# google-research/frame-interpolation

Hardware: NVIDIA H100
Metric: interpolated_frames_per_sec_1080p (higher is better)
Workload: dtype f16x2-split (activations/weights as fp16 hi+lo planes; fp32 accumulate)

## Files before the change

### frame_interpolation_b200/csrc/film_conv.h

```cpp
#pragma once
#include <cuda.h>
#include <stdint.h>

#include "film_common.cuh"

namespace film {

constexpr int kMaxSrc = 4;
constexpr int kMaxTaps = 9;
constexpr int kChunk = 64;
constexpr int kTileM = 128;

struct ConvSrc {
  const sp_t* hi;
  const sp_t* lo;
  int C;
  int c_off;
  int nchunk;
  int bswap;
};

struct alignas(64) ConvProblem {
  CUtensorMap tm_a_hi[kMaxSrc];
  CUtensorMap tm_a_lo[kMaxSrc];
  CUtensorMap tm_w_hi;
  CUtensorMap tm_w_lo;
  CUtensorMap tm_w_hi_half;
  CUtensorMap tm_w_lo_half;
  ConvSrc src[kMaxSrc];
  int nsrc;
  int B, H, W;
  int tile_h, tile_w;
  int tiles_y, tiles_x;
  int ntaps;
  int tap_dy[kMaxTaps], tap_dx[kMaxTaps];
  int kchunk;
  int ktot;
  const sp_t* w_hi;
  const sp_t* w_lo;
  const float* bias;
  int cout;
  int act;
  sp_t* out_hi;
  sp_t* out_lo;
  int out_C, out_c_off;
  int out_H, out_W;
  int out_sy, out_sx, out_oy, out_ox;
  int epi_mode;
  const float* head_w3;
  const float* head_b3;
  int crop_y, crop_x, crop_h, crop_w;
  int64_t crop_pitch;
  const float* head_w4;
  const float* head_b4;
  const float* head_vup;
  float* head_res;
  float* head_v;
  int v2_resident;
  int v2_na, v2_nw;
  int v2_grid;
  int v2_part_lo, v2_part_hi;
  sp_t* pool_hi;
  sp_t* pool_lo;
  int pool_C;
  int group;
  int pair;
  int halo;
  int bn;
  int passes;
  int straight;
  int out_lo_skip;
  int pxn;
};

cudaError_t launch_conv_tc(const ConvProblem* d_prob, const ConvProblem& h_prob, cudaStream_t st);
cudaError_t launch_conv_simt(const ConvProblem* d_prob, const ConvProblem& h_prob, cudaStream_t st);
cudaError_t conv_tc_configure();
bool conv3x3_tc_plan(ConvProblem& h_prob, int num_sms);
void conv3x3_tc_pick_tile(int H, int W, int B, int cout, int kc, int passes, int ktot, int epi_mode, int num_sms,
                          int& tile_h, int& tile_w);
cudaError_t launch_conv3x3_tc(const ConvProblem* d_prob, const ConvProblem& h_prob, cudaStream_t st);
cudaError_t conv3x3_tc_configure();
}
```

### frame_interpolation_b200/csrc/film_conv3x3_tc.cu

```cuda
#include <cuda.h>
#include <cuda_runtime.h>
#include <stdint.h>

#include <type_traits>

#include "film_conv.h"
#include "film_tc_ptx.cuh"

namespace film {
namespace {
using namespace tc;

constexpr int kConsumers = 256;
constexpr int kThreads = kConsumers + 128;
__host__ __device__ constexpr int a_plane_bytes(int kc, int th, int tw) { return (th + 2) * tw * kc * 2; }
__host__ __device__ constexpr int a_stage_bytes(int kc, int th, int tw) { return 2 * a_plane_bytes(kc, th, tw); }
constexpr int kHaloW = 10;
__host__ __device__ constexpr int halo_box_bytes(int kc, int th) { return (th + 2) * kHaloW * kc * 2; }
__host__ __device__ constexpr int halo_plane_bytes(int kc, int th) { return (halo_box_bytes(kc, th) + 1023) & ~1023; }
__host__ __device__ constexpr int a_stage_bytes_h(int kc, int th, int tw, int halo, int planes = 2) {
  return planes * (halo ? halo_plane_bytes(kc, th) : a_plane_bytes(kc, th, tw));
}
constexpr int kMaxRing = 8;
constexpr int kSmemLimit = 227 * 1024;
constexpr int kBarBytes = 8 * (4 * kMaxRing + 4);
constexpr int kFixedBytes = kBarBytes + 16 + 512 * 4  + 64  + 1024  + 64;
constexpr int kHeadW3 = 64 * 32 * 4, kHeadMisc = 512;
constexpr int kHeadBytes = kHeadW3 + kHeadMisc;
constexpr int kPxnStageWg = 64 * 64 * 2;
constexpr int kPxnStageBytes = 2 * kPxnStageWg;
constexpr int kFoldLd = 136;
constexpr int kFoldStageWg = 32 * kFoldLd * 4;
inline int epi_scratch_bytes(int epi_mode, int pxn, int bn) {
  if (pxn && bn == 32) return (epi_mode == 3 ? kHeadBytes : 0) + 2 * kFoldStageWg;
  return epi_mode == 3 ? kHeadBytes : pxn ? kPxnStageBytes : 0;
}

__host__ __device__ constexpr int w_rows(int bn, int pxn) { return pxn && bn == 32 ? 64 : bn; }
__host__ __device__ inline int w_tap_bytes(int bn, int kc, int planes = 2) { return bn * kc * 2 * planes; }

template <int BN, int KC, bool kPartial, bool kHalo, bool kOne, bool kRes, bool kPxN = false>
__global__ void __launch_bounds__(kThreads, 1) k_conv3x3_tc(const ConvProblem* __restrict__ prob) {
  static_assert(!kPxN || ((BN == 64 || BN == 128) && KC == 64) || (BN == 32 && kOne && !kPartial),
                "pixels on N: one or two M = 64 weight tiles of 64-channel chunks, or the folded single-pass Cout = 32 form");
  extern __shared__ uint8_t smem_raw[];
  constexpr bool one = kOne;
  const int planes = one ? 1 : 2;
  constexpr bool kFold = kPxN && BN == 32;
  constexpr int kWPlane = w_rows(BN, kPxN) * KC * 2;
  const int kWTap = kWPlane * planes;
  const int kTileH = prob->tile_h, kTileW = prob->tile_w;
  constexpr int kHaloTileH = kPxN ? 32 : 16;
  constexpr int kHaloBox = halo_box_bytes(KC, kHaloTileH), kHaloPlane = halo_plane_bytes(KC, kHaloTileH);
  constexpr bool halo = kHalo;
  const int kAPlane = halo ? kHaloPlane : a_plane_bytes(KC, kTileH, kTileW);
  const int kAStage = planes * kAPlane;
  const int kRowStep = kTileW * KC * 2;
  constexpr bool kFused = BN <= 128 && !kPxN;
  constexpr int kMh = kPxN && !kFold ? BN / 64 : 1;
  constexpr int kPxnN = kFold ? 136 : 128;
  constexpr int kAccRegs = kPxN ? kPxnN / 2 * kMh : (kFused ? 2 * BN : BN) / 2;
  constexpr int kWgPx = kPxN ? 128 : 64;

  const int NA = prob->v2_na, NW = prob->v2_nw;
  const bool resident = prob->v2_resident != 0;
  const int nsrc = prob->nsrc;
  const int tiles_x = prob->tiles_x, tiles_per_img = prob->tiles_y * prob->tiles_x;
  const int cout = prob->cout;
  const int n_nt = (cout + BN - 1) / BN;
  const int ntiles = prob->B * tiles_per_img * n_nt;
  constexpr int kStageTaps = kHalo ? 9 : 3;
  constexpr int kStageMmas = kFold ? 2 * kStageTaps / 3 : kStageTaps;
  constexpr bool kPacked = kPartial && kPxN;
  const int part_lo = prob->v2_part_lo, part_hi = prob->v2_part_hi;
  int nab = 0;
  for (int s = 0; s < nsrc; ++s) nab += prob->src[s].nchunk * (kHalo ? 1 : 3);
  const int nkb = nab * kStageMmas - (kPacked ? (part_hi - part_lo) * (kStageTaps - kStageTaps / 3) : 0);

  const FastDiv div_nt(n_nt, ntiles), div_img(tiles_per_img, ntiles), div_tx(tiles_x, ntiles);
  const bool pair = prob->pair != 0;
  const int rank = pair ? (int)cluster_ctarank() : 0;
  const int nsp = prob->B * tiles_per_img;
  const int nwork = pair ? ((nsp + 1) / 2) * n_nt : ntiles;
  const int w_first = pair ? (int)blockIdx.x >> 1 : (int)blockIdx.x, w_step = pair ? (int)gridDim.x >> 1 : (int)gridDim.x;
  auto decode = [&](int work, int& sp, int& nti) {
    div_nt.divmod(work, sp, nti);
    if (pair) sp = 2 * sp + rank;
  };

  const uint32_t raw = smem_u32(smem_raw);
  const uint32_t base = (raw + 1023u) & ~1023u;
  uint8_t* gen_base = smem_raw + (base - raw);
  const uint32_t a_base = base;
  const uint32_t w_base = a_base + (uint32_t)NA * kAStage;
  const uint32_t w_bytes = resident ? (uint32_t)nkb * kWTap : (uint32_t)NW * kWTap;
  const uint32_t tail = w_base + w_bytes;
  const uint32_t tail_off = (uint32_t)NA * kAStage + w_bytes;
  float* bias_smem = reinterpret_cast<float*>(gen_base + tail_off + kBarBytes + 16);
  int* src_tab = reinterpret_cast<int*>(gen_base + tail_off + kBarBytes + 16 + 512 * 4);

  const int warp = threadIdx.x >> 5, lane = threadIdx.x & 31;

  if (warp == 8 && lane == 0) {
    for (int s = 0; s < kMaxRing; ++s) {
      mbar_init(tail + 8u * s, 1);
      mbar_init(tail + 8u * (kMaxRing + s), 2);
      mbar_init(tail + 8u * (2 * kMaxRing + s), 1);
      mbar_init(tail + 8u * (3 * kMaxRing + s), pair ? 4 : 2);
    }
    for (int s = 0; s < kMaxSrc; ++s) {
      src_tab[2 * s] = s < nsrc ? prob->src[s].nchunk : 0;
      src_tab[2 * s + 1] = s < nsrc ? prob->src[s].c_off : 0;
      src_tab[2 * kMaxSrc + s] = s < nsrc ? prob->src[s].bswap : 0;
    }
    asm volatile("fence.mbarrier_init.release.cluster;" ::: "memory");
  }
  if (warp < 8)
    for (int i = threadIdx.x; i < n_nt * BN; i += kConsumers) bias_smem[i] = (i < cout) ? prob->bias[i] : 0.f;
  __syncthreads();
  if (pair) cluster_sync_all();
  auto leave = [&]() {
    if (pair) cluster_sync_all();
  };

  if (warp >= 8) {
    regs_dec<40>();
    if (warp > 8) {
      leave();
      return;
    }
    const CUtensorMap* tm_w_hi = &prob->tm_w_hi;
    const CUtensorMap* tm_w_lo = &prob->tm_w_lo;
    if (resident && elect_one()) {
      mbar_expect_tx(tail + 8u * (2 * kMaxRing), (uint32_t)nkb * kWTap);
      for (int kb = 0; kb < nkb; ++kb) {
        tma_load_2d(w_base + kb * kWTap, tm_w_hi, tail + 8u * (2 * kMaxRing), kb * KC, 0);
        if (!one) tma_load_2d(w_base + kb * kWTap + kWPlane, tm_w_lo, tail + 8u * (2 * kMaxRing), kb * KC, 0);
      }
    }
    __syncwarp();
    RingPos ra, rw;
    for (int tile = w_first; tile < nwork; tile += w_step) {
      int sp, nti, b, rem, ty, tx;
      decode(tile, sp, nti);
      div_img.divmod(sp, b, rem);
      div_tx.divmod(rem, ty, tx);
      const int n0 = nti * BN, y0 = ty * kTileH, x0 = tx * kTileW;
      {
        const int nt = tile + w_step;
        int next_sp, nnt;
        decode(nt < nwork ? nt : 0, next_sp, nnt);
        if (nt < nwork && next_sp != sp && next_sp < nsp && elect_one()) {
          int nb, nrem, nty, ntx;
          div_img.divmod(next_sp, nb, nrem);
          div_tx.divmod(nrem, nty, ntx);
          const int ny0 = nty * kTileH, nx0 = ntx * kTileW;
          for (int s = 0; s < nsrc; ++s)
            for (int ch = 0; ch < src_tab[2 * s]; ++ch) {
              const int cc = src_tab[2 * s + 1] + ch * KC;
              tma_prefetch_4d(&prob->tm_a_hi[s], cc, nx0 - 1, ny0 - 1, nb);
              if (!one) tma_prefetch_4d(&prob->tm_a_lo[s], cc, nx0 - 1, ny0 - 1, nb);
              if (!halo) {
                tma_prefetch_4d(&prob->tm_a_hi[s], cc, nx0 + 1, ny0 - 1, nb);
                if (!one) tma_prefetch_4d(&prob->tm_a_lo[s], cc, nx0 + 1, ny0 - 1, nb);
              }
            }
        }
        __syncwarp();
      }
      int kb = 0, ab = 0;
      for (int s = 0; s < nsrc; ++s) {
        const int nchunk = src_tab[2 * s], c_off = src_tab[2 * s + 1];
        const int bs = src_tab[2 * kMaxSrc + s] ? prob->B - 1 - b : b;
        const CUtensorMap* tm_hi = &prob->tm_a_hi[s];
        const CUtensorMap* tm_lo = &prob->tm_a_lo[s];
        for (int ch = 0; ch < nchunk; ++ch) {
          const int nst = halo ? 1 : 3;
          for (int dx = 0; dx < nst; ++dx, ++ab) {
            const int st = ra.stage;
            mbar_wait(tail + 8u * (kMaxRing + st), ra.phase ^ 1u);
            if (elect_one()) {
              const uint32_t sa = a_base + st * kAStage, bar = tail + 8u * st;
              mbar_expect_tx(bar, halo ? (uint32_t)(planes * kHaloBox) : (uint32_t)kAStage);
              tma_load_4d(sa, tm_hi, bar, c_off + ch * KC, x0 + dx - 1, y0 - 1, bs);
              if (!one) tma_load_4d(sa + kAPlane, tm_lo, bar, c_off + ch * KC, x0 + dx - 1, y0 - 1, bs);
            }
            __syncwarp();
            ra.advance(NA);
            if (!resident) {
              const bool packed = kPacked && ab >= part_lo && ab < part_hi;
              const int nblk = packed ? kStageTaps / 3 : kStageMmas;
              for (int t = 0; t < nblk; ++t, ++kb) {
                const int ws = rw.stage;
                mbar_wait(tail + 8u * (3 * kMaxRing + ws), rw.phase ^ 1u);
                if (elect_one()) {
                  const uint32_t sw = w_base + ws * kWTap, bar = tail + 8u * (2 * kMaxRing + ws);
                  mbar_expect_tx(bar, kWTap);
                  if (pair) {
                    const uint32_t hoff = (uint32_t)(rank * (kWPlane / 2));
                    tma_load_2d_mc(sw + hoff, &prob->tm_w_hi_half, bar, kb * KC, n0 + rank * (BN / 2), 3);
                    if (!one) tma_load_2d_mc(sw + kWPlane + hoff, &prob->tm_w_lo_half, bar, kb * KC, n0 + rank * (BN / 2), 3);
                  } else {
                    tma_load_2d(sw, tm_w_hi, bar, kb * KC, n0);
                    if (!one) tma_load_2d(sw + kWPlane, tm_w_lo, bar, kb * KC, n0);
                  }
                }
                __syncwarp();
                rw.advance(NW);
              }
            }
          }
        }
      }
    }
    leave();
    return;
  }

  regs_inc<232>();
  const int wg = warp >> 2;
  const int q = lane & 3;
  const int H = prob->H, W = prob->W, out_H = prob->out_H, out_W = prob->out_W, out_C = prob->out_C;
  const int out_c_off = prob->out_c_off, act = prob->act;
  sp_t* const out_hi = prob->out_hi;
  sp_t* const out_lo = prob->out_lo;
  sp_t* const pool_hi = prob->pool_hi;
  sp_t* const pool_lo = prob->pool_lo;
  const int pool_C = prob->pool_C;
  const bool do_pool = pool_hi != nullptr;
  const bool lo_skip = prob->out_lo_skip != 0;
  const bool rgb = prob->epi_mode == 2;
  const float* const head_w = prob->head_w4;
  float* const rgb_out = prob->head_v;
  const int crop_y = prob->crop_y, crop_x = prob->crop_x, crop_h = prob->crop_h, crop_w = prob->crop_w;
  const int64_t crop_pitch = prob->crop_pitch;
  const bool fhead = prob->epi_mode == 3;
  constexpr int kHid = BN <= 64 ? BN / 2 : 1;
  float* const w3s = reinterpret_cast<float*>(reinterpret_cast<uint8_t*>(src_tab) + 64);
  float* const hmisc = w3s + kHeadW3 / 4;
  if (fhead) {
    if constexpr (BN <= 64) {
      for (int i = threadIdx.x; i < BN * kHid; i += kConsumers) w3s[i] = prob->head_w3[i];
      for (int i = threadIdx.x; i < kHid; i += kConsumers) hmisc[i] = prob->head_b3[i];
      for (int i = threadIdx.x; i < 2 * kHid; i += kConsumers) hmisc[kHid + i] = prob->head_w4[i];
      if (threadIdx.x < 2) hmisc[3 * kHid + threadIdx.x] = prob->head_b4[threadIdx.x];
    }
    asm volatile("bar.sync 1, %0;" ::"r"(kConsumers) : "memory");
  }
  const float* const head_vup = prob->head_vup;
  float* const head_res = prob->head_res;
  float* const head_vout = prob->head_v;

  if (resident) mbar_wait(tail + 8u * (2 * kMaxRing), 0);
  const bool is_leader = (threadIdx.x & 127) == 0;
  const uint32_t w_empty_peer = pair ? map_to_cta(tail + 8u * (3 * kMaxRing), (uint32_t)(rank ^ 1)) : 0u;
  auto release_w = [&](int slot) {
    mbar_arrive(tail + 8u * (3 * kMaxRing + slot));
    if (pair) mbar_arrive_cluster(w_empty_peer + 8u * slot);
  };
  {
    constexpr int kWTapC = kWPlane * (kOne ? 1 : 2);
    constexpr uint32_t kPx = KC * 2;
    const uint32_t a_row0 = kHalo ? (uint32_t)(wg * (kWgPx / 8) * kHaloW) * kPx : (uint32_t)(wg * kWgPx) * kPx;
    const uint32_t sbo = kHalo ? kHaloW * kPx : 8 * kPx;
    RingPos ra, rw;
    float acc[kAccRegs];
    auto tap_of = [](int m) { return kFold ? (kHalo ? 3 * (m / 2) : 0) + m % 2 : m; };
    auto pxn_mma = [&](uint64_t w_hi, uint64_t w_lo, uint64_t a_hi, uint64_t a_lo, uint32_t accf) {
#pragma unroll
      for (int h = 0; h < kMh; ++h) {
        const uint64_t wh = (uint64_t)(h * (64 * KC * 2) >> 4);
        wgmma<kPxnN>(acc + 64 * h, w_hi + wh, a_hi, accf);
        if constexpr (!kOne) {
          wgmma<kPxnN>(acc + 64 * h, w_lo + wh, a_hi, 1u);
          wgmma<kPxnN>(acc + 64 * h, w_hi + wh, a_lo, 1u);
        }
      }
    };
    for (int tile = w_first; tile < nwork; tile += w_step) {
      int kb = 0;
      int rel_a = -1, rel_w = -1;
      auto retire = [&](int next_a, int next_w) {
        wgmma_commit();
        wgmma_wait<1>();
        if (is_leader) {
          if (rel_a >= 0) mbar_arrive(tail + 8u * (kMaxRing + rel_a));
          if (rel_w >= 0) release_w(rel_w);
        }
        rel_a = next_a;
        rel_w = next_w;
      };
      auto stage = [&](auto ksteps_c, auto tpb_c) {
        constexpr int kSteps = decltype(ksteps_c)::value, kTpb = decltype(tpb_c)::value;
        constexpr int kBlocks = kStageMmas / kTpb;
        const int st = ra.stage;
        mbar_wait(tail + 8u * st, ra.phase);
        const uint32_t sa = a_base + st * kAStage + a_row0;
        const uint32_t lo_off = (uint32_t)(kHalo ? kHaloPlane : kAPlane);
        if constexpr (kRes) {
          const uint64_t a0 = make_desc_sbo<KC>(sa, sbo);
          const uint64_t lo_delta = (uint64_t)(lo_off >> 4);
          const uint64_t row_delta = (uint64_t)(kRowStep >> 4);
          const uint64_t w0 = make_desc_kc<KC>(w_base + kb * kWTapC);
          const uint32_t first = (kb == 0) ? 0u : 1u;
          wgmma_fence();
#pragma unroll
          for (int mi = 0; mi < kStageMmas; ++mi) {
            const int t = tap_of(mi);
            const uint64_t a_hi = a0 + (kHalo ? (uint64_t)((((t % 3) * kHaloW + t / 3) * kPx) >> 4) : (uint64_t)t * row_delta);
            const uint64_t a_lo = a_hi + lo_delta;
            const uint64_t w_hi = w0 + (uint64_t)(((mi / kTpb) * kWTapC + (mi % kTpb) * kSteps * 32) >> 4);
            const uint64_t w_lo = w_hi + (uint64_t)(kWPlane >> 4);
#pragma unroll
            for (int k = 0; k < kSteps; ++k) {
              const uint64_t adv = (uint64_t)(k * 32 >> 4);
              const uint32_t accf = (mi == 0 && k == 0) ? first : 1u;
              if constexpr (kPxN) {
                pxn_mma(w_hi + adv, w_lo + adv, a_hi + adv, a_lo + adv, accf);
              } else if constexpr (kOne) {
                wgmma<BN>(acc, a_hi + adv, w_hi + adv, accf);
              } else if constexpr (kFused) {
                wgmma<BN>(acc, a_hi + adv, w_hi + adv, accf);
                wgmma<BN>(acc + BN / 2, a_hi + adv, w_lo + adv, accf);
                wgmma<BN>(acc, a_lo + adv, w_hi + adv, 1u);
              } else {
                wgmma<BN>(acc, a_lo + adv, w_hi + adv, accf);
                wgmma<BN>(acc, a_hi + adv, w_lo + adv, 1u);
                wgmma<BN>(acc, a_hi + adv, w_hi + adv, 1u);
              }
            }
          }
          retire(st, -1);
          kb += kBlocks;
        } else {
          for (int blk = 0; blk < kBlocks; ++blk, ++kb) {
            uint32_t sw;
            int ws = -1;
            if (resident) {
              sw = w_base + kb * kWTap;
            } else {
              ws = rw.stage;
              mbar_wait(tail + 8u * (2 * kMaxRing + ws), rw.phase);
              sw = w_base + ws * kWTap;
            }
            const uint32_t first = (kb == 0) ? 0u : 1u;
            wgmma_fence();
#pragma unroll
            for (int u = 0; u < kTpb; ++u) {
              const int t = tap_of(blk * kTpb + u);
              const uint32_t off = kHalo ? (uint32_t)((t % 3) * kHaloW + t / 3) * kPx : (uint32_t)(t * kRowStep);
              const uint64_t a_hi = make_desc_sbo<KC>(sa + off, sbo);
              const uint64_t a_lo = make_desc_sbo<KC>(sa + lo_off + off, sbo);
              const uint64_t wk = (uint64_t)((u * kSteps * 32) >> 4);
              const uint64_t w_hi = make_desc_kc<KC>(sw) + wk, w_lo = make_desc_kc<KC>(sw + kWPlane) + wk;
#pragma unroll
              for (int k = 0; k < kSteps; ++k) {
                const uint64_t adv = (uint64_t)(k * 32 >> 4);
                const uint32_t accf = (u == 0 && k == 0) ? first : 1u;
                if constexpr (kPxN) {
                  pxn_mma(w_hi + adv, w_lo + adv, a_hi + adv, a_lo + adv, accf);
                } else if constexpr (kOne) {
                  wgmma<BN>(acc, a_hi + adv, w_hi + adv, accf);
                } else if constexpr (kFused) {
                  wgmma<BN>(acc, a_hi + adv, w_hi + adv, accf);
                  wgmma<BN>(acc + BN / 2, a_hi + adv, w_lo + adv, accf);
                  wgmma<BN>(acc, a_lo + adv, w_hi + adv, 1u);
                } else {
                  wgmma<BN>(acc, a_lo + adv, w_hi + adv, accf);
                  wgmma<BN>(acc, a_hi + adv, w_lo + adv, 1u);
                  wgmma<BN>(acc, a_hi + adv, w_hi + adv, 1u);
                }
              }
            }
            retire(blk == kBlocks - 1 ? st : -1, ws);
            if (!resident) rw.advance(NW);
          }
        }
        ra.advance(NA);
      };
      using Full = std::integral_constant<int, KC / 16>;
      using One = std::integral_constant<int, 1>;
      if constexpr (kPartial) {
        for (int ab = 0; ab < part_lo; ++ab) stage(Full{}, One{});
        for (int ab = part_lo; ab < part_hi; ++ab) stage(One{}, std::integral_constant<int, kPacked ? 3 : 1>{});
        for (int ab = part_hi; ab < nab; ++ab) stage(Full{}, One{});
      } else {
        for (int ab = 0; ab < nab; ++ab) stage(Full{}, One{});
      }
      wgmma_wait<0>();
      if (is_leader) {
        if (rel_a >= 0) mbar_arrive(tail + 8u * (kMaxRing + rel_a));
        if (rel_w >= 0) release_w(rel_w);
      }
      acc_fence<kAccRegs>(acc);

      int sp, nti, b, rem, ty, tx;
      decode(tile, sp, nti);
      div_img.divmod(sp, b, rem);
      div_tx.divmod(rem, ty, tx);
      const int n0 = nti * BN;
      const bool live = sp < nsp;
      if constexpr (kFold) {
        float* const stg = reinterpret_cast<float*>(reinterpret_cast<uint8_t*>(src_tab) + 64 + (fhead ? kHeadBytes : 0) +
                                                    wg * kFoldStageWg);
        auto wg_sync = [&]() { asm volatile("bar.sync %0, 128;" ::"r"(2 + wg) : "memory"); };
        const bool lower = (warp & 2) != 0;
        const int r0 = 16 * (warp & 1) + (lane >> 2);
        wg_sync();
        if (!lower) {
#pragma unroll
          for (int j = 0; j < 16; ++j)
#pragma unroll
            for (int h = 0; h < 2; ++h)
              *reinterpret_cast<float2*>(stg + (r0 + 8 * h) * kFoldLd + 8 * j + 2 * q) =
                  make_float2(acc[4 * j + 2 * h], acc[4 * j + 2 * h + 1]);
        }
        wg_sync();
        if (lower) {
#pragma unroll
          for (int j = 1; j < 17; ++j)
#pragma unroll
            for (int h = 0; h < 2; ++h) {
              float2* d = reinterpret_cast<float2*>(stg + (r0 + 8 * h) * kFoldLd + 8 * (j - 1) + 2 * q);
              const float2 v = *d;
              *d = make_float2(v.x + acc[4 * j + 2 * h], v.y + acc[4 * j + 2 * h + 1]);
            }
        }
        wg_sync();
        const int p = threadIdx.x & 127;
        const int py = ty * kTileH + 16 * wg + (p >> 3), px = tx * kTileW + (p & 7);
        const int64_t opix = ((int64_t)b * out_H + py) * out_W + px;
        float f[32];
#pragma unroll
        for (int c = 0; c < 32; ++c) {
          const float x = stg[c * kFoldLd + p] + bias_smem[c];
          f[c] = act ? leaky(x) : x;
        }
        if (!live || py >= H || px >= W) {
        } else if (fhead) {
          float hp[16];
#pragma unroll
          for (int hh = 0; hh < 16; ++hh) hp[hh] = 0.f;
#pragma unroll
          for (int c = 0; c < 32; ++c) {
            const float4* wr = reinterpret_cast<const float4*>(w3s + c * 16);
#pragma unroll
            for (int h4 = 0; h4 < 4; ++h4) {
              const float4 wv = wr[h4];
              hp[4 * h4] = fmaf(f[c], wv.x, hp[4 * h4]);
              hp[4 * h4 + 1] = fmaf(f[c], wv.y, hp[4 * h4 + 1]);
              hp[4 * h4 + 2] = fmaf(f[c], wv.z, hp[4 * h4 + 2]);
              hp[4 * h4 + 3] = fmaf(f[c], wv.w, hp[4 * h4 + 3]);
            }
          }
          float f0 = hmisc[3 * 16], f1 = hmisc[3 * 16 + 1];
#pragma unroll
          for (int hh = 0; hh < 16; ++hh) {
            const float x = leaky(hp[hh] + hmisc[hh]);
            f0 = fmaf(x, hmisc[16 + 2 * hh], f0);
            f1 = fmaf(x, hmisc[16 + 2 * hh + 1], f1);
          }
          float2 res = make_float2(f0, f1), tot = res;
          if (head_vup) {
            const float2 u = reinterpret_cast<const float2*>(head_vup)[opix];
            tot.x += u.x;
            tot.y += u.y;
          }
          reinterpret_cast<float2*>(head_res)[opix] = res;
// ... 153 lines not shown
            for (int e = 0; e < 2; ++e) {
              const int c = n0 + 8 * j + 2 * q + e;
              float f = value(h, j, e) + bias_smem[c];
              if (act) f = leaky(f);
              r0 = fmaf(f, __ldg(head_w + 3 * c), r0);
              r1 = fmaf(f, __ldg(head_w + 3 * c + 1), r1);
              r2 = fmaf(f, __ldg(head_w + 3 * c + 2), r2);
            }
#pragma unroll
          for (int m = 1; m <= 2; m <<= 1) {
            r0 += __shfl_xor_sync(0xffffffffu, r0, m);
            r1 += __shfl_xor_sync(0xffffffffu, r1, m);
            r2 += __shfl_xor_sync(0xffffffffu, r2, m);
          }
          const int oy = py - crop_y, ox = px - crop_x;
          if (q == 0 && valid && oy >= 0 && oy < crop_h && ox >= 0 && ox < crop_w) {
            float* o = rgb_out + (int64_t)oy * crop_pitch + (int64_t)ox * 3;
            o[0] = r0 + __ldg(prob->head_b4);
            o[1] = r1 + __ldg(prob->head_b4 + 1);
            o[2] = r2 + __ldg(prob->head_b4 + 2);
          }
        }
      }
      if (!fhead && !rgb) {
        bool valid[2];
        int64_t opix[2];
#pragma unroll
        for (int h = 0; h < 2; ++h) {
          const int r = wg * 64 + (warp & 3) * 16 + (lane >> 2) + 8 * h;
          const int py = ty * kTileH + r / kTileW, px = tx * kTileW + r % kTileW;
          valid[h] = live && (py < H) && (px < W);
          opix[h] = ((int64_t)b * out_H + py) * out_W + px;
        }
        const int r0 = wg * 64 + (warp & 3) * 16 + (lane >> 2);
        const int py0 = ty * kTileH + r0 / kTileW, px0 = tx * kTileW + r0 % kTileW;
        const bool pool_ok = live && (py0 >> 1) < (out_H >> 1) && (px0 >> 1) < (out_W >> 1) && !(lane & 4);
        const int64_t ppix = ((int64_t)b * (out_H >> 1) + (py0 >> 1)) * (out_W >> 1) + (px0 >> 1);
#pragma unroll
        for (int j = 0; j < BN / 8; ++j) {
          const int c = 8 * j + 2 * q;
          if (n0 + c >= cout) break;
          float a[2][2];
#pragma unroll
          for (int h = 0; h < 2; ++h) {
            float f0 = value(h, j, 0) + bias_smem[n0 + c], f1 = value(h, j, 1) + bias_smem[n0 + c + 1];
            if (act) {
              f0 = leaky(f0);
              f1 = leaky(f1);
            }
            if (valid[h]) {
              sp_t* oh = out_hi + opix[h] * out_C + out_c_off + n0;
              if (lo_skip) {
                *reinterpret_cast<uint32_t*>(oh + c) = pack2_hi(f0, f1);
              } else {
                sp_t* ol = out_lo + opix[h] * out_C + out_c_off + n0;
                uint32_t hi, lo;
                split_pack2(f0, f1, hi, lo);
                *reinterpret_cast<uint32_t*>(oh + c) = hi;
                *reinterpret_cast<uint32_t*>(ol + c) = lo;
              }
            }
            if (do_pool) {
              a[h][0] = f0 + __shfl_xor_sync(0xffffffffu, f0, 4);
              a[h][1] = f1 + __shfl_xor_sync(0xffffffffu, f1, 4);
            }
          }
          if (do_pool && pool_ok) {
            uint32_t hi, lo;
            split_pack2((a[0][0] + a[1][0]) * 0.25f, (a[0][1] + a[1][1]) * 0.25f, hi, lo);
            *reinterpret_cast<uint32_t*>(pool_hi + ppix * pool_C + n0 + c) = hi;
            *reinterpret_cast<uint32_t*>(pool_lo + ppix * pool_C + n0 + c) = lo;
          }
        }
      }
    }
  }
  leave();
}

int smem_bytes_for(const ConvProblem& h, int bn) {
  const int nkb = h.ktot / h.kchunk;
  const int planes = h.passes == 1 ? 1 : 2;
  const int wtap = w_tap_bytes(w_rows(bn, h.pxn), h.kchunk, planes);
  const int w = h.v2_resident ? nkb * wtap : h.v2_nw * wtap;
  return h.v2_na * a_stage_bytes_h(h.kchunk, h.tile_h, h.tile_w, h.halo, planes) + w + kFixedBytes +
         epi_scratch_bytes(h.epi_mode, h.pxn, bn);
}

}

int conv_tc_block_n(int cout);

namespace {
bool ring_depths(int kc, int tile_h, int tile_w, int halo, int planes, int bn, int cout, int ktot, int epi_mode, int pxn,
                 int& resident, int& na, int& nw) {
  const int wtap = w_tap_bytes(w_rows(bn, pxn), kc, planes);
  const int w_all = (ktot / kc) * wtap;
  const int kLimit = kSmemLimit - epi_scratch_bytes(epi_mode, pxn, bn);
  const int kAStage = a_stage_bytes_h(kc, tile_h, tile_w, halo, planes);
  if (cout <= bn && w_all + 2 * kAStage + kFixedBytes <= kLimit) {
    resident = 1;
    const int n = (kLimit - kFixedBytes - w_all) / kAStage;
    const int n_max = halo ? 3 : 6;
    na = n > n_max ? n_max : n;
    nw = 1;
    return true;
  }
  resident = 0;
  na = halo ? 2 : (bn >= 128 ? 2 : 3);
  int n = (kLimit - kFixedBytes - na * kAStage) / wtap;
  if (n < 2 && na > 2) {
    na = 2;
    n = (kLimit - kFixedBytes - na * kAStage) / wtap;
  }
  nw = n > kMaxRing ? kMaxRing : n;
  return nw >= 2;
}
}

void conv3x3_tc_pick_tile(int H, int W, int B, int cout, int kc, int passes, int ktot, int epi_mode, int num_sms,
                          int& tile_h, int& tile_w) {
  static const int cand[3][2] = {{16, 8}, {8, 16}, {4, 32}};
  const int bn = conv_tc_block_n(cout);
  const int n_nt = (cout + bn - 1) / bn;
  double best = 1e30;
  tile_h = 16;
  tile_w = 8;
  for (auto& c : cand) {
    int res, na, nw;
    if (!ring_depths(kc, c[0], c[1], 0, passes == 1 ? 1 : 2, bn, cout, ktot, epi_mode, 0, res, na, nw)) continue;
    const long tiles = (long)B * ((H + c[0] - 1) / c[0]) * ((W + c[1] - 1) / c[1]) * n_nt;
    const long waves = (tiles + num_sms - 1) / num_sms;
    const double cost = (double)waves * (c[0] + 2.0) / c[0] * (1.0 + 1e-3 * (c[1] / 8));
    if (cost < best) {
      best = cost;
      tile_h = c[0];
      tile_w = c[1];
    }
  }
}

bool conv3x3_tc_plan(ConvProblem& h, int num_sms) {
  const int bn = h.bn;
  const int planes = h.passes == 1 ? 1 : 2;
  const int wtap = w_tap_bytes(w_rows(bn, h.pxn), h.kchunk, planes);
  const int w_all = (h.ktot / h.kchunk) * wtap;
  const bool can_resident = h.cout <= bn;
  const int kLimit = kSmemLimit - epi_scratch_bytes(h.epi_mode, h.pxn, bn);
  if (h.halo && (h.tile_h != (h.pxn ? 32 : 16) || h.tile_w != 8 ||
                 (can_resident && w_all + 2 * a_stage_bytes_h(h.kchunk, h.tile_h, h.tile_w, 0, planes) + kFixedBytes <= kLimit &&
                  w_all + 2 * a_stage_bytes_h(h.kchunk, h.tile_h, h.tile_w, 1, planes) + kFixedBytes > kLimit)))
    h.halo = 0;
  bool ok = ring_depths(h.kchunk, h.tile_h, h.tile_w, h.halo, planes, bn, h.cout, h.ktot, h.epi_mode, h.pxn,
                        h.v2_resident, h.v2_na, h.v2_nw);
  if (!ok && h.halo) {
    h.halo = 0;
    ok = ring_depths(h.kchunk, h.tile_h, h.tile_w, 0, planes, bn, h.cout, h.ktot, h.epi_mode, h.pxn, h.v2_resident,
                     h.v2_na, h.v2_nw);
  }
  const int nsp = h.B * h.tiles_y * h.tiles_x, n_nt = (h.cout + bn - 1) / bn;
  if (h.pair) {
    const int nwork = (nsp + 1) / 2 * n_nt, nclu = num_sms / 2;
    h.v2_grid = 2 * (nwork < nclu ? nwork : nclu);
  } else {
    h.v2_grid = nsp * n_nt < num_sms ? nsp * n_nt : num_sms;
  }
  return ok;
}

using ConvKernel = void (*)(const ConvProblem*);
template <int BN, int KC, bool kPartial, bool kHalo, bool kOne, bool kRes, bool kPxN>
constexpr ConvKernel kernel_of() {
  if constexpr (kPxN && BN == 32 && (kPartial || !kOne))
    return nullptr;
  else
    return k_conv3x3_tc<BN, KC, kPartial, kHalo, kOne, kRes, kPxN>;
}

template <int BN, int KC, bool kPxN = false>
struct Variants {
  static constexpr ConvKernel kFn[16] = {
      kernel_of<BN, KC, false, false, false, false, kPxN>(), kernel_of<BN, KC, false, false, false, true, kPxN>(),
      kernel_of<BN, KC, false, false, true, false, kPxN>(),  kernel_of<BN, KC, false, false, true, true, kPxN>(),
      kernel_of<BN, KC, false, true, false, false, kPxN>(),  kernel_of<BN, KC, false, true, false, true, kPxN>(),
      kernel_of<BN, KC, false, true, true, false, kPxN>(),   kernel_of<BN, KC, false, true, true, true, kPxN>(),
      kernel_of<BN, KC, true, false, false, false, kPxN>(),  kernel_of<BN, KC, true, false, false, true, kPxN>(),
      kernel_of<BN, KC, true, false, true, false, kPxN>(),   kernel_of<BN, KC, true, false, true, true, kPxN>(),
      kernel_of<BN, KC, true, true, false, false, kPxN>(),   kernel_of<BN, KC, true, true, false, true, kPxN>(),
      kernel_of<BN, KC, true, true, true, false, kPxN>(),    kernel_of<BN, KC, true, true, true, true, kPxN>()};
  static cudaError_t configure() {
    for (auto fn : kFn) {
      if (!fn) continue;
      const cudaError_t e = cudaFuncSetAttribute(fn, cudaFuncAttributeMaxDynamicSharedMemorySize, kSmemLimit);
      if (e != cudaSuccess) return e;
    }
    return cudaSuccess;
  }
  static cudaError_t launch(const ConvProblem* d_prob, const ConvProblem& h, cudaStream_t st) {
    if (h.v2_na < 2 || (!h.v2_resident && h.v2_nw < 2)) return cudaErrorInvalidValue;
    if (kPxN && (h.pair || h.tile_h != 32 || h.tile_w != 8 || h.epi_mode != (BN == 32 && h.epi_mode == 3 ? 3 : 0)))
      return cudaErrorInvalidValue;
    if (kPxN && BN == 32 && h.pool_hi) return cudaErrorInvalidValue;
    const bool partial = h.v2_part_hi > h.v2_part_lo;
    const int idx = (partial ? 8 : 0) | (h.halo ? 4 : 0) | (h.passes == 1 ? 2 : 0) | (h.v2_resident && h.straight ? 1 : 0);
    if (!kFn[idx]) return cudaErrorInvalidValue;
    if (!h.pair) {
      kFn[idx]<<<h.v2_grid, kThreads, smem_bytes_for(h, BN), st>>>(d_prob);
      return cudaGetLastError();
    }
    cudaLaunchConfig_t cfg = {};
    cudaLaunchAttribute attr[1];
    attr[0].id = cudaLaunchAttributeClusterDimension;
    attr[0].val.clusterDim.x = 2;
    attr[0].val.clusterDim.y = 1;
    attr[0].val.clusterDim.z = 1;
    cfg.gridDim = dim3(h.v2_grid);
    cfg.blockDim = dim3(kThreads);
    cfg.dynamicSmemBytes = smem_bytes_for(h, BN);
    cfg.stream = st;
    cfg.attrs = attr;
    cfg.numAttrs = 1;
    return cudaLaunchKernelEx(&cfg, kFn[idx], d_prob);
  }
};

cudaError_t conv3x3_tc_configure() {
  cudaError_t e;
#define FILM_CFG(BN, KC)                        \
  e = Variants<BN, KC>::configure();            \
  if (e != cudaSuccess) return e;
  FILM_CFG(32, 64) FILM_CFG(64, 64) FILM_CFG(128, 64) FILM_CFG(256, 64) FILM_CFG(32, 32) FILM_CFG(64, 32)
#undef FILM_CFG
  e = Variants<64, 64, true>::configure();
  if (e != cudaSuccess) return e;
  e = Variants<128, 64, true>::configure();
  if (e != cudaSuccess) return e;
  e = Variants<32, 64, true>::configure();
  if (e != cudaSuccess) return e;
  e = Variants<32, 32, true>::configure();
  if (e != cudaSuccess) return e;
  return cudaSuccess;
}

cudaError_t launch_conv3x3_tc(const ConvProblem* d_prob, const ConvProblem& h, cudaStream_t st) {
  const int bn = h.bn;
  if (h.kchunk == 32) {
    if (bn == 32) return h.pxn ? Variants<32, 32, true>::launch(d_prob, h, st) : Variants<32, 32>::launch(d_prob, h, st);
    if (bn == 64) return Variants<64, 32>::launch(d_prob, h, st);
    return cudaErrorInvalidValue;
  }
  switch (bn) {
    case 256: return Variants<256, 64>::launch(d_prob, h, st);
    case 128: return h.pxn ? Variants<128, 64, true>::launch(d_prob, h, st) : Variants<128, 64>::launch(d_prob, h, st);
    case 64: return h.pxn ? Variants<64, 64, true>::launch(d_prob, h, st) : Variants<64, 64>::launch(d_prob, h, st);
    default: return h.pxn ? Variants<32, 64, true>::launch(d_prob, h, st) : Variants<32, 64>::launch(d_prob, h, st);
  }
}

}
```

### frame_interpolation_b200/csrc/film_kernels.cu

```cuda
#include "film_conv.h"
#include "film_kernels.h"

namespace film {

static inline int cdiv(int64_t a, int64_t b) { return (int)((a + b - 1) / b); }

__device__ __forceinline__ uint4 ldg16(const void* p) { return __ldg(reinterpret_cast<const uint4*>(p)); }

__global__ void k_image_pool(const float* __restrict__ in, float* __restrict__ out, int B, int H,
                             int W) {
  const int Ho = H / 2, Wo = W / 2;
  const int64_t n = (int64_t)B * Ho * Wo * 3;
  int64_t i = (int64_t)blockIdx.x * blockDim.x + threadIdx.x;
  if (i >= n) return;
  int c = (int)(i % 3);
  int64_t p = i / 3;
  int x = (int)(p % Wo);
  p /= Wo;
  int y = (int)(p % Ho);
  int b = (int)(p / Ho);
  const float* r0 = in + (((int64_t)b * H + 2 * y) * W + 2 * x) * 3 + c;
  const float* r1 = r0 + (int64_t)W * 3;
  out[i] = (r0[0] + r0[3] + r1[0] + r1[3]) * 0.25f;
}
// ... 185 lines not shown
  float acc[8];
#pragma unroll
  for (int j = 0; j < 8; ++j) acc[j] = 0.f;
#pragma unroll
  for (int ky = 0; ky < 3; ++ky) {
    int yy = y + ky - 1;
    if (yy < 0 || yy >= H) continue;
#pragma unroll
    for (int kx = 0; kx < 3; ++kx) {
      int xx = x + kx - 1;
      if (xx < 0 || xx >= W) continue;
      const float* ip = img + (((int64_t)b * H + yy) * W + xx) * 3;
#pragma unroll
      for (int ci = 0; ci < 3; ++ci) {
        float v = __ldg(ip + ci);
        const float* wr = ws + ((ky * 3 + kx) * 3 + ci) * 64 + g * 8;
#pragma unroll
        for (int j = 0; j < 8; ++j) acc[j] = fmaf(v, wr[j], acc[j]);
      }
    }
  }
#pragma unroll
  for (int j = 0; j < 8; ++j) acc[j] = leaky(acc[j] + bs[g * 8 + j]);
  uint4 h, l;
  pack8(acc, h, l);
  int64_t o = p * out_C + out_c_off + g * 8;
  *reinterpret_cast<uint4*>(out_hi + o) = h;
  *reinterpret_cast<uint4*>(out_lo + o) = l;
}

constexpr int kC0H = 8, kC0W = 16;
constexpr int kC0Tiles = 4;
constexpr int kC0Patch = (kC0H + 2) * (kC0W + 2) * 3;
constexpr int kC0PatchRegs = (kC0Patch + 127) / 128;
__device__ __forceinline__ float fe_patch_load(const float* __restrict__ img, int b, int H, int W, int y0, int x0, int i) {
  const int c = i % 3, px = (i / 3) % (kC0W + 2), py = i / (3 * (kC0W + 2));
  const int yy = y0 + py - 1, xx = x0 + px - 1;
  return (i < kC0Patch && yy >= 0 && yy < H && xx >= 0 && xx < W) ? __ldg(img + (((int64_t)b * H + yy) * W + xx) * 3 + c) : 0.f;
}
__global__ void __launch_bounds__(128) k_fe_conv0(const float* __restrict__ img, int H, int W,
                                                  const float* __restrict__ w, const float* __restrict__ bias,
                                                  sp_t* __restrict__ out_hi, sp_t* __restrict__ out_lo, int lo_skip,
                                                  float* __restrict__ pool_out) {
  __shared__ float4 ws[27 * 16];
  __shared__ float bs[64];
  __shared__ float patch[kC0Patch];
  const int tid = threadIdx.x;
  const int b = blockIdx.z, y0 = blockIdx.y * kC0H, xb = blockIdx.x * (kC0W * kC0Tiles);
  for (int i = tid; i < 27 * 16; i += 128) ws[i] = __ldg(reinterpret_cast<const float4*>(w) + i);
  if (tid < 64) bs[tid] = bias[tid];
  float nxt[kC0PatchRegs];
#pragma unroll
  for (int j = 0; j < kC0PatchRegs; ++j) nxt[j] = fe_patch_load(img, b, H, W, y0, xb, tid + 128 * j);
  const int warp = tid >> 5, lane = tid & 31;
  const int r = lane >> 2, cx = (lane & 3) * 4;
  const int y = y0 + r;
#pragma unroll 1
  for (int tile = 0; tile < kC0Tiles; ++tile) {
    const int x0 = xb + tile * kC0W;
    if (x0 >= W) break;
    __syncthreads();
#pragma unroll
    for (int j = 0; j < kC0PatchRegs; ++j)
      if (tid + 128 * j < kC0Patch) patch[tid + 128 * j] = nxt[j];
    __syncthreads();
    if (pool_out != nullptr && tid < (kC0H / 2) * (kC0W / 2) * 3) {
      const int c = tid % 3, qx = (tid / 3) % (kC0W / 2), qy = tid / (3 * (kC0W / 2));
      const int oy = (y0 >> 1) + qy, ox = (x0 >> 1) + qx;
      if (oy < (H >> 1) && ox < (W >> 1)) {
        const float* p0 = patch + ((2 * qy + 1) * (kC0W + 2) + 2 * qx + 1) * 3 + c;
        const float* p1 = p0 + (kC0W + 2) * 3;
        pool_out[(((int64_t)b * (H >> 1) + oy) * (W >> 1) + ox) * 3 + c] = (p0[0] + p0[3] + p1[0] + p1[3]) * 0.25f;
      }
    }
    if (tile + 1 < kC0Tiles && x0 + kC0W < W) {
#pragma unroll
      for (int j = 0; j < kC0PatchRegs; ++j) nxt[j] = fe_patch_load(img, b, H, W, y0, x0 + kC0W, tid + 128 * j);
    }
    float acc[4][16];
#pragma unroll
    for (int p = 0; p < 4; ++p)
#pragma unroll
      for (int j = 0; j < 16; ++j) acc[p][j] = 0.f;
#pragma unroll
    for (int ky = 0; ky < 3; ++ky) {
      float in[18];
      const float* pr = patch + ((r + ky) * (kC0W + 2) + cx) * 3;
#pragma unroll
      for (int j = 0; j < 18; ++j) in[j] = pr[j];
#pragma unroll
      for (int kx = 0; kx < 3; ++kx)
#pragma unroll
        for (int ci = 0; ci < 3; ++ci) {
          const float4* wk = ws + ((ky * 3 + kx) * 3 + ci) * 16 + warp * 4;
          const float4 w0 = wk[0], w1 = wk[1], w2 = wk[2], w3 = wk[3];
          const float wv[16] = {w0.x, w0.y, w0.z, w0.w, w1.x, w1.y, w1.z, w1.w, w2.x, w2.y, w2.z, w2.w, w3.x, w3.y, w3.z, w3.w};
#pragma unroll
          for (int p = 0; p < 4; ++p) {
            const float v = in[(p + kx) * 3 + ci];
#pragma unroll
            for (int j = 0; j < 16; ++j) acc[p][j] = fmaf(v, wv[j], acc[p][j]);
          }
        }
    }
    if (y < H) {
#pragma unroll
      for (int p = 0; p < 4; ++p) {
        const int x = x0 + cx + p;
        if (x < W) {
          float f[16];
#pragma unroll
          for (int j = 0; j < 16; ++j) f[j] = leaky(acc[p][j] + bs[warp * 16 + j]);
          const int64_t o = (((int64_t)b * H + y) * W + x) * 64 + warp * 16;
          if (lo_skip) pack_store16_hi(f, out_hi + o);
          else pack_store16(f, out_hi + o, out_lo + o);
        }
      }
    }
  }
}
cudaError_t launch_fe_conv0(const float* img, int B, int H, int W, const float* w, const float* bias, sp_t* out_hi,
                            sp_t* out_lo, bool lo_skip, float* pool_out, cudaStream_t st) {
  dim3 grid((W + kC0W * kC0Tiles - 1) / (kC0W * kC0Tiles), (H + kC0H - 1) / kC0H, B);
  k_fe_conv0<<<grid, 128, 0, st>>>(img, H, W, w, bias, out_hi, out_lo, lo_skip ? 1 : 0, pool_out);
  return cudaGetLastError();
}

cudaError_t launch_conv0_c3(const float* img, int B, int H, int W, const float* w,
                            const float* bias, sp_t* out_hi, sp_t* out_lo, int out_C,
                            int out_c_off, cudaStream_t st) {
  int64_t npix = (int64_t)B * H * W;
  k_conv0_c3<<<cdiv(npix, 32), 256, 0, st>>>(img, B, H, W, w, bias, out_hi, out_lo, out_C, out_c_off);
  return cudaGetLastError();
}

__global__ void __launch_bounds__(256) k_im2col3x3(const float* __restrict__ img, int B, int H, int W,
                                                   sp_t* __restrict__ out_hi, sp_t* __restrict__ out_lo) {
  const int64_t n = (int64_t)B * H * W * 4;
  int64_t i = (int64_t)blockIdx.x * blockDim.x + threadIdx.x;
  if (i >= n) return;
  const int g = (int)(i & 3);
  const int64_t p = i >> 2;
  const int x = (int)(p % W);
  const int64_t q = p / W;
  const int y = (int)(q % H);
  const int b = (int)(q / H);
  float v[8];
#pragma unroll
  for (int j = 0; j < 8; ++j) {
    const int k = g * 8 + j;
    float val = 0.f;
    if (k < 27) {
      const int tap = k / 3, ci = k - tap * 3;
      const int yy = y + tap / 3 - 1, xx = x + tap % 3 - 1;
      if (yy >= 0 && yy < H && xx >= 0 && xx < W) val = __ldg(img + (((int64_t)b * H + yy) * W + xx) * 3 + ci);
    }
    v[j] = val;
  }
  uint4 h, l;
  pack8(v, h, l);
  *reinterpret_cast<uint4*>(out_hi + p * 32 + g * 8) = h;
  *reinterpret_cast<uint4*>(out_lo + p * 32 + g * 8) = l;
}

__global__ void __launch_bounds__(256) k_image_to_split32(const float* __restrict__ img, int64_t npix,
                                                          sp_t* __restrict__ out_hi, sp_t* __restrict__ out_lo) {
  int64_t p = (int64_t)blockIdx.x * blockDim.x + threadIdx.x;
// ... 564 lines not shown
```

Baseline: 28.44.

## Add split-plane conv3x3 variant with resident hi weights and streamed lo weights

Adds a kSplit variant of the pixels-on-N 3x3 tensor-core conv for single-source, BN=64, halo, two-pass layers. The hi weight plane for all nine taps is loaded once and kept resident in shared memory, and only the lo weight plane is streamed through a ring. Activation hi and lo are loaded as separate single-plane halo boxes: hi×(w_hi+w_lo) runs first, then lo×w_hi against the resident weights. This shrinks the per-stage A footprint and weight traffic in exchange for a more serialized activation schedule. It also stops unrolling the ky loop in the first feature-extraction conv, likely to reduce register pressure.

```diff
diff --git a/frame_interpolation_b200/csrc/film_conv.h b/frame_interpolation_b200/csrc/film_conv.h
--- a/frame_interpolation_b200/csrc/film_conv.h
+++ b/frame_interpolation_b200/csrc/film_conv.h
@@ -58,6 +58,7 @@
   float* head_v;
   int v2_resident;
   int v2_na, v2_nw;
+  int v2_split;
   int v2_grid;
   int v2_part_lo, v2_part_hi;
   sp_t* pool_hi;
diff --git a/frame_interpolation_b200/csrc/film_conv3x3_tc.cu b/frame_interpolation_b200/csrc/film_conv3x3_tc.cu
--- a/frame_interpolation_b200/csrc/film_conv3x3_tc.cu
+++ b/frame_interpolation_b200/csrc/film_conv3x3_tc.cu
@@ -39,10 +39,12 @@
 __host__ __device__ constexpr int w_rows(int bn, int pxn) { return pxn && bn == 32 ? 64 : bn; }
 __host__ __device__ inline int w_tap_bytes(int bn, int kc, int planes = 2) { return bn * kc * 2 * planes; }
 
-template <int BN, int KC, bool kPartial, bool kHalo, bool kOne, bool kRes, bool kPxN = false>
+template <int BN, int KC, bool kPartial, bool kHalo, bool kOne, bool kRes, bool kPxN = false, bool kSplit = false>
 __global__ void __launch_bounds__(kThreads, 1) k_conv3x3_tc(const ConvProblem* __restrict__ prob) {
   static_assert(!kPxN || ((BN == 64 || BN == 128) && KC == 64) || (BN == 32 && kOne && !kPartial),
                 "pixels on N: one or two M = 64 weight tiles of 64-channel chunks, or the folded single-pass Cout = 32 form");
+  static_assert(!kSplit || (kPxN && BN == 64 && kHalo && !kOne && !kPartial && !kRes),
+                "split planes: three-pass pixels on N, BN = 64, wide halo, every k-step issued");
   extern __shared__ uint8_t smem_raw[];
   constexpr bool one = kOne;
   const int planes = one ? 1 : 2;
@@ -54,7 +56,7 @@
   constexpr int kHaloBox = halo_box_bytes(KC, kHaloTileH), kHaloPlane = halo_plane_bytes(KC, kHaloTileH);
   constexpr bool halo = kHalo;
   const int kAPlane = halo ? kHaloPlane : a_plane_bytes(KC, kTileH, kTileW);
-  const int kAStage = planes * kAPlane;
+  const int kAStage = (kSplit ? 1 : planes) * kAPlane;
   const int kRowStep = kTileW * KC * 2;
   constexpr bool kFused = BN <= 128 && !kPxN;
   constexpr int kMh = kPxN && !kFold ? BN / 64 : 1;
@@ -93,9 +95,11 @@
   uint8_t* gen_base = smem_raw + (base - raw);
   const uint32_t a_base = base;
   const uint32_t w_base = a_base + (uint32_t)NA * kAStage;
-  const uint32_t w_bytes = resident ? (uint32_t)nkb * kWTap : (uint32_t)NW * kWTap;
+  const uint32_t w_bytes = kSplit ? (uint32_t)(nkb + NW) * kWPlane : resident ? (uint32_t)nkb * kWTap : (uint32_t)NW * kWTap;
+  const uint32_t w_lo_ring = w_base + (uint32_t)nkb * kWPlane;
   const uint32_t tail = w_base + w_bytes;
   const uint32_t tail_off = (uint32_t)NA * kAStage + w_bytes;
+  const uint32_t w_hi_full = tail + 8u * (4 * kMaxRing);
   float* bias_smem = reinterpret_cast<float*>(gen_base + tail_off + kBarBytes + 16);
   int* src_tab = reinterpret_cast<int*>(gen_base + tail_off + kBarBytes + 16 + 512 * 4);
 
@@ -108,6 +112,7 @@
       mbar_init(tail + 8u * (2 * kMaxRing + s), 1);
       mbar_init(tail + 8u * (3 * kMaxRing + s), pair ? 4 : 2);
     }
+    mbar_init(w_hi_full, 1);
     for (int s = 0; s < kMaxSrc; ++s) {
       src_tab[2 * s] = s < nsrc ? prob->src[s].nchunk : 0;
       src_tab[2 * s + 1] = s < nsrc ? prob->src[s].c_off : 0;
@@ -137,6 +142,10 @@
         tma_load_2d(w_base + kb * kWTap, tm_w_hi, tail + 8u * (2 * kMaxRing), kb * KC, 0);
         if (!one) tma_load_2d(w_base + kb * kWTap + kWPlane, tm_w_lo, tail + 8u * (2 * kMaxRing), kb * KC, 0);
       }
+    }
+    if (kSplit && elect_one()) {
+      mbar_expect_tx(w_hi_full, (uint32_t)nkb * kWPlane);
+      for (int kb = 0; kb < nkb; ++kb) tma_load_2d(w_base + kb * kWPlane, tm_w_hi, w_hi_full, kb * KC, 0);
     }
     __syncwarp();
     RingPos ra, rw;
@@ -167,6 +176,33 @@
             }
         }
         __syncwarp();
+      }
+      if constexpr (kSplit) {
+        auto load_box = [&](const CUtensorMap* tm) {
+          const int st = ra.stage;
+          mbar_wait(tail + 8u * (kMaxRing + st), ra.phase ^ 1u);
+          if (elect_one()) {
+            const uint32_t bar = tail + 8u * st;
+            mbar_expect_tx(bar, (uint32_t)kHaloBox);
+            tma_load_4d(a_base + st * kAStage, tm, bar, src_tab[1], x0 - 1, y0 - 1, src_tab[2 * kMaxSrc] ? prob->B - 1 - b : b);
+          }
+          __syncwarp();
+          ra.advance(NA);
+        };
+        load_box(&prob->tm_a_hi[0]);
+        for (int kb = 0; kb < nkb; ++kb) {
+          const int ws = rw.stage;
+          mbar_wait(tail + 8u * (3 * kMaxRing + ws), rw.phase ^ 1u);
+          if (elect_one()) {
+            const uint32_t bar = tail + 8u * (2 * kMaxRing + ws);
+            mbar_expect_tx(bar, (uint32_t)kWPlane);
+            tma_load_2d(w_lo_ring + ws * kWPlane, tm_w_lo, bar, kb * KC, n0);
+          }
+          __syncwarp();
+          rw.advance(NW);
+        }
+        load_box(&prob->tm_a_lo[0]);
+        continue;
       }
       int kb = 0, ab = 0;
       for (int s = 0; s < nsrc; ++s) {
@@ -252,6 +288,7 @@
   float* const head_vout = prob->head_v;
 
   if (resident) mbar_wait(tail + 8u * (2 * kMaxRing), 0);
+  if (kSplit) mbar_wait(w_hi_full, 0);
   const bool is_leader = (threadIdx.x & 127) == 0;
   const uint32_t w_empty_peer = pair ? map_to_cta(tail + 8u * (3 * kMaxRing), (uint32_t)(rank ^ 1)) : 0u;
   auto release_w = [&](int slot) {
@@ -384,6 +421,39 @@
         for (int ab = 0; ab < part_lo; ++ab) stage(Full{}, One{});
         for (int ab = part_lo; ab < part_hi; ++ab) stage(One{}, std::integral_constant<int, kPacked ? 3 : 1>{});
         for (int ab = part_hi; ab < nab; ++ab) stage(Full{}, One{});
+      } else if constexpr (kSplit) {
+        const int st_hi = ra.stage;
+        mbar_wait(tail + 8u * st_hi, ra.phase);
+        ra.advance(NA);
+        const uint32_t sa_hi = a_base + st_hi * kAStage + a_row0;
+        for (int t = 0; t < 9; ++t) {
+          const int ws = rw.stage;
+          mbar_wait(tail + 8u * (2 * kMaxRing + ws), rw.phase);
+          const uint64_t a = make_desc_sbo<KC>(sa_hi + (uint32_t)((t % 3) * kHaloW + t / 3) * kPx, sbo);
+          const uint64_t wh = make_desc_kc<KC>(w_base + t * kWPlane), wl = make_desc_kc<KC>(w_lo_ring + ws * kWPlane);
+          wgmma_fence();
+#pragma unroll
+          for (int k = 0; k < KC / 16; ++k) {
+            const uint64_t adv = (uint64_t)(k * 32 >> 4);
+            wgmma<kPxnN>(acc, wh + adv, a + adv, (t == 0 && k == 0) ? 0u : 1u);
+            wgmma<kPxnN>(acc, wl + adv, a + adv, 1u);
+          }
+          retire(t == 8 ? st_hi : -1, ws);
+          rw.advance(NW);
+        }
+        const int st_lo = ra.stage;
+        mbar_wait(tail + 8u * st_lo, ra.phase);
+        ra.advance(NA);
+        const uint64_t a0 = make_desc_sbo<KC>(a_base + st_lo * kAStage + a_row0, sbo);
+        const uint64_t w0 = make_desc_kc<KC>(w_base);
+        wgmma_fence();
+#pragma unroll
+        for (int t = 0; t < 9; ++t)
+#pragma unroll
+          for (int k = 0; k < KC / 16; ++k)
+            wgmma<kPxnN>(acc, w0 + (uint64_t)((t * kWPlane + k * 32) >> 4),
+                         a0 + (uint64_t)((((t % 3) * kHaloW + t / 3) * kPx + k * 32) >> 4), 1u);
+        retire(st_lo, -1);
       } else {
         for (int ab = 0; ab < nab; ++ab) stage(Full{}, One{});
       }
@@ -703,8 +773,8 @@
   const int nkb = h.ktot / h.kchunk;
   const int planes = h.passes == 1 ? 1 : 2;
   const int wtap = w_tap_bytes(w_rows(bn, h.pxn), h.kchunk, planes);
-  const int w = h.v2_resident ? nkb * wtap : h.v2_nw * wtap;
-  return h.v2_na * a_stage_bytes_h(h.kchunk, h.tile_h, h.tile_w, h.halo, planes) + w + kFixedBytes +
+  const int w = h.v2_split ? (nkb + h.v2_nw) * w_tap_bytes(bn, h.kchunk, 1) : h.v2_resident ? nkb * wtap : h.v2_nw * wtap;
+  return h.v2_na * a_stage_bytes_h(h.kchunk, h.tile_h, h.tile_w, h.halo, h.v2_split ? 1 : planes) + w + kFixedBytes +
          epi_scratch_bytes(h.epi_mode, h.pxn, bn);
 }
 
@@ -779,6 +849,17 @@
     ok = ring_depths(h.kchunk, h.tile_h, h.tile_w, 0, planes, bn, h.cout, h.ktot, h.epi_mode, h.pxn, h.v2_resident,
                      h.v2_na, h.v2_nw);
   }
+  h.v2_split = 0;
+  if (ok && h.pxn && bn == 64 && h.cout <= 64 && planes == 2 && h.halo && !h.v2_resident && !h.pair && h.nsrc == 1 &&
+      h.kchunk == 64 && h.ktot == 9 * h.kchunk) {
+    const int plane = a_stage_bytes_h(h.kchunk, h.tile_h, h.tile_w, 1, 1), wplane = w_tap_bytes(bn, h.kchunk, 1);
+    const int nw = (kLimit - kFixedBytes - 2 * plane - 9 * wplane) / wplane;
+    if (nw >= 2) {
+      h.v2_split = 1;
+      h.v2_na = 2;
+      h.v2_nw = nw > kMaxRing ? kMaxRing : nw;
+    }
+  }
   const int nsp = h.B * h.tiles_y * h.tiles_x, n_nt = (h.cout + bn - 1) / bn;
   if (h.pair) {
     const int nwork = (nsp + 1) / 2 * n_nt, nclu = num_sms / 2;
@@ -796,6 +877,13 @@
     return nullptr;
   else
     return k_conv3x3_tc<BN, KC, kPartial, kHalo, kOne, kRes, kPxN>;
+}
+template <int BN, int KC, bool kPxN>
+constexpr ConvKernel split_kernel_of() {
+  if constexpr (kPxN && BN == 64 && KC == 64)
+    return k_conv3x3_tc<BN, KC, false, true, false, false, true, true>;
+  else
+    return nullptr;
 }
 
 template <int BN, int KC, bool kPxN = false>
@@ -809,12 +897,14 @@
       kernel_of<BN, KC, true, false, true, false, kPxN>(),   kernel_of<BN, KC, true, false, true, true, kPxN>(),
       kernel_of<BN, KC, true, true, false, false, kPxN>(),   kernel_of<BN, KC, true, true, false, true, kPxN>(),
       kernel_of<BN, KC, true, true, true, false, kPxN>(),    kernel_of<BN, KC, true, true, true, true, kPxN>()};
+  static constexpr ConvKernel kSplitFn = split_kernel_of<BN, KC, kPxN>();
   static cudaError_t configure() {
     for (auto fn : kFn) {
       if (!fn) continue;
       const cudaError_t e = cudaFuncSetAttribute(fn, cudaFuncAttributeMaxDynamicSharedMemorySize, kSmemLimit);
       if (e != cudaSuccess) return e;
     }
+    if (kSplitFn) return cudaFuncSetAttribute(kSplitFn, cudaFuncAttributeMaxDynamicSharedMemorySize, kSmemLimit);
     return cudaSuccess;
   }
   static cudaError_t launch(const ConvProblem* d_prob, const ConvProblem& h, cudaStream_t st) {
@@ -824,9 +914,10 @@
     if (kPxN && BN == 32 && h.pool_hi) return cudaErrorInvalidValue;
     const bool partial = h.v2_part_hi > h.v2_part_lo;
     const int idx = (partial ? 8 : 0) | (h.halo ? 4 : 0) | (h.passes == 1 ? 2 : 0) | (h.v2_resident && h.straight ? 1 : 0);
-    if (!kFn[idx]) return cudaErrorInvalidValue;
+    const ConvKernel fn = h.v2_split ? (idx == 4 ? kSplitFn : nullptr) : kFn[idx];
+    if (!fn) return cudaErrorInvalidValue;
     if (!h.pair) {
-      kFn[idx]<<<h.v2_grid, kThreads, smem_bytes_for(h, BN), st>>>(d_prob);
+      fn<<<h.v2_grid, kThreads, smem_bytes_for(h, BN), st>>>(d_prob);
       return cudaGetLastError();
     }
     cudaLaunchConfig_t cfg = {};
@@ -841,7 +932,7 @@
     cfg.stream = st;
     cfg.attrs = attr;
     cfg.numAttrs = 1;
-    return cudaLaunchKernelEx(&cfg, kFn[idx], d_prob);
+    return cudaLaunchKernelEx(&cfg, fn, d_prob);
   }
 };
 
diff --git a/frame_interpolation_b200/csrc/film_kernels.cu b/frame_interpolation_b200/csrc/film_kernels.cu
--- a/frame_interpolation_b200/csrc/film_kernels.cu
+++ b/frame_interpolation_b200/csrc/film_kernels.cu
@@ -291,7 +291,7 @@
     for (int p = 0; p < 4; ++p)
 #pragma unroll
       for (int j = 0; j < 16; ++j) acc[p][j] = 0.f;
-#pragma unroll
+#pragma unroll 1
     for (int ky = 0; ky < 3; ++ky) {
       float in[18];
       const float* pr = patch + ((r + ky) * (kC0W + 2) + cx) * 3;
```

Result: faster. 30.40 (median of 6 runs) (+6.9%).
